# Hippogriff/prifit

Measured on AMD Instinct MI355X. Metric: shapes/sec (fwd+bwd) B=24x2048 pts, PointNet++-MSG+ellipsoid fit, higher is better.
Workload: dtype f32; 1 GPU; configs[2]: PointNet++-MSG + mean-shift(10 it, <=25 clusters) + ellipsoid fit + convex loss, B=24x2048 per GPU, fwd+bwd+Adam; global_batch=24, points=2048, parallelism=dp1, cloud=blobs, embedding=clustered, backbone_grad_param=sa1.conv_blocks.0.0.weight, launch=eager

## Files before the change

include/prifit_hip.h:

```cpp
#ifndef PRIFIT_HIP_H
#define PRIFIT_HIP_H

#include <stdint.h>

#ifdef __cplusplus
extern "C" {
#endif

#define PRIFIT_OK 0
#define PRIFIT_EINVAL (-1)
#define PRIFIT_ELAUNCH (-2)

#define PRIFIT_ABI_VERSION 802
int prifit_version(const char **arch);


int prifit_fps(const float *xyz, int B, int N, int npoint, const int64_t *start_idx,
               int64_t *out_idx, float *new_xyz, void *stream);

int prifit_ball_query(const float *xyz, const float *new_xyz, int B, int N, int S, int R,
                      const float *radius2, const int *nsample, void *const *out, int idx64,
                      void *stream);

int prifit_three_nn(const float *xyz1, const float *xyz2, int B, int N, int S, int32_t *idx,
                    float *dist, float *weight, void *stream);

int prifit_square_distance(const float *src, const float *dst, int B, int S, int N, float *out,
                           void *stream);


int prifit_group_gather(const float *feat, const float *xyz, const float *new_xyz,
                        const int32_t *idx, int B, int N, int S, int K, int C, int order,
                        int ld_out, float *out, void *stream);

int prifit_group_scatter_add(const float *gout, int ld_gout, int col0, const int32_t *idx, int B,
                             int N, int S, int K, int C, float *dfeat, void *stream);

int prifit_pack_cols(const float *w, int rows, int src_cols, const int32_t *map, int dst_cols, float *out, void *stream);
int prifit_unpack_cols(const float *g, int rows, int dst_cols, const int32_t *inv_off, const int32_t *inv_idx, int src_cols,
                       float *gw, void *stream);
int prifit_pack_cols_max_jobs(void);
int prifit_pack_cols_multi(int njobs, const float *const *w, const int32_t *rows, const int32_t *src_cols, const int32_t *const *map,
                           const int32_t *dst_cols, float *const *out, void *stream);
int prifit_unpack_cols_multi(int njobs, const float *const *g, const int32_t *rows, const int32_t *dst_cols, const int32_t *const *inv_off,
                             const int32_t *const *inv_idx, const int32_t *src_cols, float *const *gw, void *stream);

int prifit_three_interpolate(const float *points2, const int32_t *idx, const float *weight, int B,
                             int N, int S, int C, int ld_out, int col0, float *out, void *stream);

int prifit_three_interpolate_bwd(const float *gout, int ld_gout, int col0, const int32_t *idx,
                                 const float *weight, int B, int N, int S, int C, float *dpoints2,
                                 void *stream);
int prifit_fp_rows(const float *points2, const int32_t *idx, const float *weight, const float *points1, int B, int N, int S, int D2,
                   int D1, int kp, float *out, void *stream);


#define PRIFIT_GEMM_NT 0
#define PRIFIT_GEMM_NN 1
#define PRIFIT_GEMM_TN 2
#define PRIFIT_EPI_NONE 0
#define PRIFIT_EPI_CHORD 1
#define PRIFIT_EPI_MSKERNEL 2
#define PRIFIT_EPI_MSBWD 3

int prifit_gemm_f32(int layout, int M, int N, int K, const float *A, long long lda, long long strideA,
                    const float *B, long long ldb, long long strideB, float *C, long long ldc,
                    long long strideC, int batch, int splitk, const float *a_scale,
                    const float *a_shift, const float *b_scale, const float *b_shift,
                    const float *bias, long long bias_batch_stride, float *col_stats, int epilogue,
                    const float *epi_batch_scalar, const float *epi_aux, long long ld_aux,
                    long long stride_aux, const float *epi_row_add, float *a_rowsum, int accumulate, void *stream);

int prifit_chord_sym_f32(const float *A, long long lda, long long strideA, float *C, long long ldc, long long strideC,
                         int n, int K, int batch, unsigned long long *owner_key, void *stream);
int prifit_chord_sym_mask(const float *A, long long lda, long long strideA, const float *thr, uint32_t *mask, int n, int K, int batch,
                          unsigned long long *owner_key, void *stream);
int prifit_gram_sym_f32(const float *A, long long lda, long long strideA, float *C, long long ldc, long long strideC, int n, int K,
                        int batch, void *stream);

int prifit_gemm_pool_f32(int M, int N, int K, const float *A, long long lda, const float *W, long long ldb, float *Y,
                         long long ldc, const float *a_scale, const float *a_shift, const float *bias, float *col_stats,
                         float *cand, void *stream);
int prifit_gemm_pool_supported(int M, int N, int K);

int prifit_gemm_stream_f32(int layout, int M, int N, int K, const float *A, long long lda, const float *B,
                           long long ldb, float *C, long long ldc, const float *a_scale, const float *a_shift,
                           const float *bias, float *col_stats, void *stream);
int prifit_gemm_stream_supported(int layout, int M, int N, int K);
int prifit_gemm_stream_slabs(int M, int K);

int prifit_gemm_dual_nn_f32(int M, int N, int K1, int K2, const float *A1, const float *A2, long long lda,
                            long long strideA, const float *B1, const float *B2, long long ldb, long long strideB,
                            float *C, long long ldc, long long strideC, int batch, int splitk, int accumulate,
                            void *stream);

int prifit_gemm_dgrad_bnred_f32(int M, int N, int K, const float *dY, long long lda, const float *W, long long ldb,
// ... 334 lines not shown
long long prifit_chamfer_nn_workspace_floats(int B, int NA, int NB);
int prifit_chamfer_nn_fwd(const float *a, const float *b, const int32_t *na, const int32_t *nb, int B, int NA, int NB,
                          float *d2, int32_t *idx, float *workspace, void *stream);
int prifit_chamfer_nn_bwd(const float *a, const float *b, const int32_t *na, const int32_t *nb, int B, int NA, int NB,
                          const int32_t *idx, const float *g, float *ga, float *gb, int accumulate_b, void *stream);

long long prifit_atlas_workspace_floats(int num_charts, int B, int P, int backward);
int prifit_atlas_fwd(const void *const *params, const float *z, const float *grid, int num_charts, int B, int P, int training,
                     float eps, float momentum, float *out, float *workspace, void *stream);
int prifit_atlas_bwd(const void *const *params, const float *z, const float *grid, int num_charts, int B, int P, int training,
                     const float *gout, const float *out, const float *fwd_workspace, float *workspace, float *gz,
                     float *gparams, void *stream);


int prifit_knn_topk(const float *G, const float *xx, int B, int N, int k, int32_t *idx, void *stream);
int prifit_knn3_supported(int N, int k);
int prifit_knn3_topk(const float *x, int B, int N, int k, int32_t *idx, void *stream);

int prifit_edge_gather(const float *x, const int32_t *idx, int B, int N, int C, int k, int ld_out,
                       float *out, void *stream);
int prifit_edge_scatter(const float *gout, int ld_gout, const int32_t *idx, int B, int N, int C, int k,
                        float *dx, void *stream);

int prifit_comm_unique_id_bytes(void);
int prifit_comm_in_process(void);
int prifit_comm_unique_id(void *out);
int prifit_comm_init(void **comm, int nranks, int rank, const void *unique_id);
int prifit_allreduce_flat(float *buf, long long count, void *comm, void *stream);
int prifit_comm_destroy(void *comm);

int prifit_adam_flat_alignment(void);
int prifit_adam_flat(float *params, float *exp_avg, float *exp_avg_sq, const float *const *grads, const int32_t *offsets,
                     const int32_t *lengths, int nparams, long long total, const int32_t *step_in, int32_t *step_out, float lr,
                     float beta1, float beta2, float eps, float weight_decay, const int32_t *skip, void *stream);
int prifit_sgd_flat(float *params, float *momentum_buf, const float *const *grads, const int32_t *offsets, const int32_t *lengths,
                    int nparams, long long total, const int32_t *step_in, int32_t *step_out, float lr, float momentum,
                    float dampening, float weight_decay, int nesterov, const int32_t *skip, void *stream);

int prifit_affine_points(const float *src, int B, int M, int C, const float *affine, const int32_t *subset, int n_subset,
                         float *dst_cl, float *dst_cf, float *dst_sub, void *stream);

int prifit_seg_metrics(const float *scores, long long ld, const long long *target, int B, int N, int P,
                       const int32_t *cat_of_label, int restricted, long long *pred, int32_t *shape_cat, int32_t *inter,
                       int32_t *uni, long long *totals, void *stream);


int prifit_fold_bn_max_jobs(void);
int prifit_fold_bn(int njobs, const float *const *W, const int32_t *cout, const int32_t *kin, const float *const *bias,
                   const float *const *gamma, const float *const *beta, const float *const *mean, const float *const *var,
                   const float *eps, const long long *w_off, const int32_t *ldw, const long long *b_off, float *flat,
                   long long flat_len, void *stream);

int prifit_mlp_chain_pool_supported(int C0, int C1, int C2, int pool_K);
long long prifit_mlp_chain_pool_workspace(int G, int pool_K, int C0, int C1, int C2);
int prifit_mlp_chain_pool_f32(const float *X, long long ldx, int G, int pool_K, int C0, int C1, int C2, const float *W1,
                              long long ldw1, const float *b1, const float *W2, long long ldw2, const float *b2, float *out,
                              long long ldo, float *workspace, void *stream);

int prifit_mlp_chain_rows_supported(int K0, int L, const int32_t *widths);
long long prifit_mlp_chain_rows_workspace(long long P, int K0, int L, const int32_t *widths);
int prifit_mlp_chain_rows_f32(const float *X, long long ldx, long long P, int K0, int L, const int32_t *widths,
                              const float *const *W, const long long *ldw, const float *const *b, float *scores, long long lds,
                              int32_t *labels, const int32_t *cat_of_label, const int32_t *shape_cat, int rows_per_shape,
                              float *workspace, void *stream);


int prifit_pack_bf16_max_jobs(void);
int prifit_pack_bf16_multi(int njobs, const float *const *w, const int32_t *rows, const int32_t *cols, const int32_t *ldw,
                           const int32_t *order, uint16_t *const *out, void *stream);

int prifit_mlp_chain_pool_bf16_supported(int C0, int C1, int C2, int pool_K);
long long prifit_mlp_chain_pool_bf16_workspace(int G, int pool_K, int C0, int C1, int C2);
int prifit_mlp_chain_pool_bf16(const float *X, long long ldx, int G, int pool_K, int C0, int C1, int C2, const uint16_t *W1,
                               long long ldw1, const float *b1, const uint16_t *W2, long long ldw2, const float *b2, float *out,
                               long long ldo, float *workspace, void *stream);

int prifit_mlp_chain_rows_bf16_supported(int K0, int L, const int32_t *widths);
long long prifit_mlp_chain_rows_bf16_workspace(long long P, int K0, int L, const int32_t *widths);
int prifit_mlp_chain_rows_bf16(const float *X, long long ldx, long long P, int K0, int L, const int32_t *widths,
                               const uint16_t *const *W, const long long *ldw, const float *const *b, float *scores, long long lds,
                               int32_t *labels, const int32_t *cat_of_label, const int32_t *shape_cat, int rows_per_shape,
                               float *workspace, void *stream);

#ifdef __cplusplus
}
#endif
#endif
```

prifit_amd/build.py:

```python
import os
import subprocess
import sys
from concurrent.futures import ThreadPoolExecutor

HERE = os.path.dirname(os.path.abspath(__file__))
ROOT = os.path.dirname(HERE)
CSRC = os.path.join(HERE, "csrc")
LIBDIR = os.path.join(HERE, "lib")
LIB = os.path.join(LIBDIR, "libprifit_hip.so")
OBJDIR = os.path.join(HERE, "build")
ARCH = "gfx950"

SOURCES = {
    "pointops.hip": ["-ffp-contract=off"],
    "sa_group.hip": ["-ffp-contract=off"],
    "gemm.hip": [],
    "gemm_stream.hip": [],
    "gemm_stream_bwd.hip": [],
    "pool_alg.hip": [],
    "sa_gather_bwd.hip": [],
    "bn.hip": [],
    "meanshift.hip": [],
    "meanshift_fused.hip": [],
    "meanshift_rows.hip": [],
    "meanshift_split.hip": [],
    "fit.hip": [],
    "fit_glue.hip": [],
    "chamfer.hip": ["-ffp-contract=off"],
    "atlas.hip": [],
    "optim.hip": [],
    "augment.hip": ["-ffp-contract=off"],
    "seg_metrics.hip": [],
    "infer.hip": [],
    "infer_bf16.hip": [],
    "edge_conv.hip": [],
    "dgcnn.hip": ["-ffp-contract=off"],
    "comm.hip": [],
}
COMMON = ["-O3", "-std=c++17", "-fPIC", "--offload-arch=" + ARCH, "-I" + os.path.join(ROOT, "include"),
          "-I" + CSRC, "-Wall", "-Wno-unused-function"] + os.environ.get("PRIFIT_BUILD_DEFS", "").split()


def _hipcc():
    for c in (os.environ.get("HIPCC"), "/opt/rocm/bin/hipcc", "hipcc"):
        if c and (os.path.isabs(c) and os.path.exists(c) or not os.path.isabs(c)):
            return c
    raise RuntimeError("hipcc not found")


def _stale(target, deps):
    if not os.path.exists(target):
        return True
    t = os.path.getmtime(target)
    return any(os.path.getmtime(d) > t for d in deps)


def build_library(force=False, verbose=False):
    import fcntl
    os.makedirs(LIBDIR, exist_ok=True)
    os.makedirs(OBJDIR, exist_ok=True)
    with open(os.path.join(LIBDIR, ".build.lock"), "w") as lock:
        fcntl.flock(lock, fcntl.LOCK_EX)
        try:
            return _build_locked(force, verbose)
        finally:
            fcntl.flock(lock, fcntl.LOCK_UN)


def _build_locked(force, verbose):
    headers = [os.path.join(CSRC, f) for f in os.listdir(CSRC) if f.endswith(".h")]
    headers.append(os.path.join(ROOT, "include", "prifit_hip.h"))
    hipcc = _hipcc()
    jobs = []
    objs = []
    for src, extra in SOURCES.items():
        s = os.path.join(CSRC, src)
        o = os.path.join(OBJDIR, src.replace(".hip", ".o"))
        objs.append(o)
        if force or _stale(o, [s] + headers):
            jobs.append([hipcc] + COMMON + extra + ["-c", s, "-o", o])

    def run(cmd):
        if verbose:
            print(" ".join(cmd), flush=True)
        r = subprocess.run(cmd, capture_output=True, text=True)
        if r.returncode != 0:
            raise RuntimeError("hipcc failed:\n%s\n%s" % (" ".join(cmd), r.stderr))
        if verbose and r.stderr.strip():
            print(r.stderr)

    if jobs:
        with ThreadPoolExecutor(max_workers=min(4, len(jobs))) as ex:
            list(ex.map(run, jobs))
    if jobs or force or _stale(LIB, objs):
        tmp = LIB + ".tmp.%d" % os.getpid()
        run([hipcc, "-shared", "-fPIC", "--offload-arch=" + ARCH, "-o", tmp] + objs + ["-ldl"])
        os.replace(tmp, LIB)
    return LIB


if __name__ == "__main__":
    print(build_library(force="--force" in sys.argv, verbose=True))
```

prifit_amd/nn_ops.py:

```python
import collections
import ctypes
import os
import types

import torch

from . import profiler
from . import arena as zero_pool
from ._lib import call, cur_stream, dll, ptr, query

NT, NN, TN = 0, 1, 2
EPI_NONE, EPI_CHORD, EPI_MSKERNEL, EPI_MSBWD = 0, 1, 2, 3
_LL = ctypes.c_longlong
_F = ctypes.c_float
_D = ctypes.c_double


def _rows_per_slab():
    return query("prifit_reduce_rows_per_slab")


_STREAM = os.environ.get("PRIFIT_GEMM_STREAM", "1") != "0"
_FUSE_RED = os.environ.get("PRIFIT_FUSE_BN_REDUCE", "1") != "0"
_FUSE_POOL_FWD = os.environ.get("PRIFIT_FUSE_POOL_FWD", "1") != "0"
# ... 200 lines not shown
             ptr(sc1), ptr(sh1), ptr(mu1), ptr(is1), ptr(rslab), cur_stream())
    return G_prev, ly.dW, rslab, None


def _route_direct0(ly, route):
    if not ly.need_dW:
        return None, None, None, None
    P, Cout, G, fe, dev = ly.P, ly.Cout, ly.G, ly.front, ly.dev
    nblk = int(max(1, min(1024, (P + 1023) // 1024)))
    part = torch.empty(nblk, Cout, fe.D + 3, dtype=torch.float32, device=dev)
    if route.kernel == "gather":
        with profiler.span("sa_first_layer_dw", 4.0 * P * (Cout + 1)):
            call("prifit_sa_first_layer_dw_bn_gather", ptr(G), ptr(fe.U), ptr(fe.Vc), ptr(ly.scale), ptr(ly.shift),
                 ptr(ly.ca), ptr(ly.cb), ptr(ly.cd), ptr(fe.idx), ptr(fe.xyz), ptr(fe.new_xyz),
                 ptr(fe.feat), fe.B, fe.N, fe.S, fe.K, Cout, fe.D, int(fe.feat_first), nblk, ptr(part), cur_stream())
    else:
        with profiler.span("sa_first_layer_dw", 4.0 * P * (2 * Cout + 1)):
            call("prifit_sa_first_layer_dw_bn", ptr(G), ptr(ly.Y), ptr(ly.scale), ptr(ly.shift), ptr(ly.ca), ptr(ly.cb), ptr(ly.cd),
                 ptr(fe.idx), ptr(fe.xyz), ptr(fe.new_xyz), ptr(fe.feat), fe.B, fe.N, fe.S, fe.K, Cout,
                 fe.D, int(fe.feat_first), nblk, ptr(part), cur_stream())
    return None, slab_sum(part), None, None


def _route_gather0(ly, route):
    P, Cout, G, fe, dev = ly.P, ly.Cout, ly.G, ly.front, ly.dev
    Bq, Nq, Sq, Kq = fe.B, fe.N, fe.S, fe.K
    if route.kernel == "csr":
        Uq, Vq = fe.U.detach().contiguous(), fe.Vc.detach().contiguous()
        E = Sq * Kq
        offs = torch.empty(Bq, Nq + 1, dtype=torch.int32, device=dev)
        lst, pos, own = (torch.empty(Bq, E, dtype=torch.int32, device=dev) for _ in range(3))
        wsd = torch.empty(query("prifit_gather_linear_bwd_csr_workspace", Bq, Sq, Kq, Cout), dtype=torch.float64, device=dev)
        dU = torch.empty(Bq, Nq, Cout, dtype=torch.float32, device=dev)
        dVc = torch.empty(Bq, Sq, Cout, dtype=torch.float32, device=dev)
        with profiler.span("gather_linear_bwd", 4.0 * (2.0 * P * Cout + 4.0 * P + 2.0 * (Bq * Nq + Bq * Sq) * Cout)):
            call("prifit_list_csr", ptr(fe.idx), Bq, Nq, E, ptr(offs), ptr(lst), ptr(pos), ptr(own), cur_stream())
            call("prifit_gather_linear_bwd_csr", ptr(G), ptr(Uq), ptr(Vq), ptr(ly.bias0), ptr(ly.scale), ptr(ly.shift),
                 ptr(ly.ca), ptr(ly.cb), ptr(ly.cd), ptr(fe.idx), ptr(offs), ptr(lst), ptr(own), Bq, Nq, Sq, Kq, Cout, ptr(dU),
                 ptr(dVc), ptr(wsd), cur_stream())
    else:
        dU = zero_pool.zeros(Bq, Nq, Cout, device=dev)
        dVc = zero_pool.zeros(Bq, Sq, Cout, device=dev)
        with profiler.span("gather_linear_bwd", 4.0 * (2.0 * P * Cout + P + (Bq * Nq + Bq * Sq) * Cout)):
            call("prifit_gather_linear_bwd_bn", ptr(G), ptr(ly.Y), ptr(ly.scale), ptr(ly.shift), ptr(ly.ca), ptr(ly.cb), ptr(ly.cd),
                 ptr(fe.idx), Bq, Nq, Sq, Kq, Cout, ptr(dU), ptr(dVc), cur_stream())
    return None, dU, None, dVc


def _route_plain(ly, route):
    P, Cout, Kin, G, W, Yp, dev = ly.P, ly.Cout, ly.Kin, ly.G, ly.W, ly.Yp, ly.dev
    dY = torch.empty(P, Cout, dtype=torch.float32, device=dev)
    if ly.pooled:
        call("prifit_pool_bwd_apply", ptr(G), _LL(G.stride(0)), ptr(ly.Y), _LL(Cout), ptr(ly.arg), ptr(ly.scale), ptr(ly.shift),
             ptr(ly.ca), ptr(ly.cb), ptr(ly.cd), P // ly.pool_K, ly.pool_K, Cout, 0, _F(0.0), ptr(dY), _LL(Cout), cur_stream())
    else:
        call("prifit_bn_relu_bwd_apply", ptr(G), _LL(G.stride(0)), ptr(ly.Y), _LL(Cout), ptr(ly.scale), ptr(ly.shift),
             ptr(ly.ca), ptr(ly.cb), ptr(ly.cd), P, Cout, 0, _F(0.0), ptr(dY), _LL(Cout), cur_stream())
    if route.name == "preact0":
        return dY, None, None, None
    dW = _weight_grad(dY, P, Cout, Yp, Kin, ly.aff_p, out=ly.dW) if ly.need_dW else None
    db = dY.sum(dim=0) if ly.want_db else None
    G_prev = None if route.kernel is None else torch.empty(P, Kin, dtype=torch.float32, device=dev)
    rslab = None
    if route.red:
        (sc1, sh1), (mu1, is1) = ly.aff_p, ly.stats_p
    if route.kernel == "gemm":
        gemm(NN, P, Kin, Cout, dY, Cout, W, Kin, G_prev, Kin)
    elif route.kernel == "stream":
        rslab = torch.empty(query("prifit_gemm_stream_slabs", P, Cout), 2, Kin, dtype=torch.float32, device=dev)
        with profiler.span(profiler.tag("gemm_stream_nn", P, Kin, Cout, 0), 4.0 * (P * Cout + 2 * P * Kin + Kin * Cout)):
            call("prifit_gemm_stream_dgrad_f32", P, Kin, Cout, ptr(dY), _LL(Cout), ptr(W), _LL(Kin), ptr(G_prev),
                 _LL(Kin), ptr(Yp), _LL(Yp.stride(0)), ptr(sc1), ptr(sh1), ptr(mu1), ptr(is1), ptr(rslab), cur_stream())
    elif route.kernel == "tiled":
        t = query("prifit_gemm_stats_tile_m", P, Kin)
        rslab = torch.empty((P + t - 1) // t, 2, Kin, dtype=torch.float32, device=dev)
        with profiler.span(profiler.tag("gemm_nn_bn%d" % _bn_tile(Kin), P, Kin, Cout, "red"), 2.0 * P * Kin * Cout):
            call("prifit_gemm_dgrad_bnred_f32", P, Kin, Cout, ptr(dY), _LL(Cout), ptr(W), _LL(Kin), ptr(G_prev),
                 _LL(Kin), ptr(Yp), _LL(Yp.stride(0)), ptr(sc1), ptr(sh1), ptr(mu1), ptr(is1), ptr(rslab), cur_stream())
    return G_prev, dW, rslab, db


_ROUTES = {"pool": _route_pool, "bn": _route_bn, "norows": _fused_bwd, "direct0": _route_direct0,
           "gather0": _route_gather0, "preact0": _route_plain, "plain": _route_plain}


def _eval_coeffs(gamma, beta, rmean, rvar, eps):
    invstd = torch.rsqrt(rvar + eps)
    mean = rmean.clone()
    scale = gamma * invstd
    return scale, beta - mean * scale, mean, invstd


FrontEnd = collections.namedtuple("FrontEnd", "mode slab idx B N S K D xyz new_xyz feat feat_first U Vc",
                                  defaults=(None,) * 12)


def _mlp_tensors(convs, bns, first_weight):
    ts = []
    for i, (conv, bn) in enumerate(zip(convs, bns)):
        w = first_weight if i == 0 else conv.weight.reshape(conv.weight.shape[0], -1)
        ts += [w, conv.bias, bn.weight, bn.bias, bn.running_mean, bn.running_var]
    return ts


def front_end_args(cfg, convs, bns, front):
    cfg["front"] = front
    if front.mode == "gather":
        return cfg, _mlp_tensors(convs, bns, front.U) + [front.Vc]
    if front.mode in ("direct", "norows"):
        return cfg, _mlp_tensors(convs, bns, convs[0].weight.reshape(convs[0].weight.shape[0], -1))
    ts = _mlp_tensors(convs, bns, None)
    ts[1] = None
    return cfg, ts


class SharedMLPFn(torch.autograd.Function):

    @staticmethod
    def forward(ctx, x, cfg, *tensors):
        L = len(tensors) // 6
        front = cfg.get("front")
        mode = "plain" if front is None else front.mode
        nr = front if mode == "norows" else None
        if nr is not None:
            P, dev = nr.B * nr.S * nr.K, nr.U.device
        else:
            P, K0 = x.shape
            dev = x.device
        training = cfg["training"]
        Ys, affines, stats_saved, Ws = [], [], [], []
        prev, prev_aff = x, None
        cand = None
        for l in range(L):
            W, b, gamma, beta, rmean, rvar = tensors[6 * l:6 * l + 6]
            preact = l == 0 and front is not None
            if preact:
                W, Cout, Kin, Y = None, (nr.U.shape[-1] if nr is not None else x.shape[1]), 0, x
            else:
                W = W.contiguous()
                Cout, Kin = W.shape
                assert Kin == (nr.U.shape[-1] if (l == 1 and nr is not None) else prev.shape[1]), (Kin, l)
                Y = torch.empty(P, Cout, dtype=torch.float32, device=dev)
            if preact:
                slab = front.slab
            elif not training:
                gemm(NT, P, Cout, Kin, prev, prev.stride(0), W, Kin, Y, Cout, a_affine=prev_aff, bias=b)
            elif l == 1 and nr is not None:
                slab = torch.empty(query("prifit_gemm_stream_slabs", P, Kin), 2, Cout, dtype=torch.float32, device=dev)
                with profiler.span(profiler.tag("gemm_stream_nt", P, Cout, Kin, "gather"), 4.0 * (P * Cout + P + Cout * Kin)):
                    call("prifit_gemm_stream_gather_f32", P, Cout, ptr(nr.idx), ptr(nr.U), ptr(nr.Vc), nr.N, nr.S,
                         nr.K, ptr(W), _LL(Kin), ptr(Y), _LL(Cout), ptr(prev_aff[0]), ptr(prev_aff[1]), ptr(b), ptr(slab),
                         cur_stream())
            else:
                aligned = prev.stride(0) % 4 == 0 and prev.data_ptr() % 16 == 0 and W.data_ptr() % 16 == 0
                tile_m = query("prifit_gemm_stats_tile_m", P, Cout)
                nslab = gemm_stats_slabs(P, Cout, Kin) if aligned else (P + tile_m - 1) // tile_m
                slab = torch.empty(nslab, 2, Cout, dtype=torch.float32, device=dev)
                kernel = _forward_kernel(l == L - 1, cfg["pool_K"], aligned, prev_aff is not None, P, Cout, Kin)
                if kernel == "gemm":
                    gemm(NT, P, Cout, Kin, prev, prev.stride(0), W, Kin, Y, Cout, a_affine=prev_aff, bias=b, stats=slab)
                else:
                    cand = torch.empty(P // 32, 4, Cout, dtype=torch.float32, device=dev)
                    if kernel == "stream_pool":
                        with profiler.span(profiler.tag("gemm_stream_nt", P, Cout, Kin, 1), 4.0 * (P * Kin + P * Cout + Cout * Kin)):
                            call("prifit_gemm_stream_pool_f32", P, Cout, Kin, ptr(prev), _LL(prev.stride(0)), ptr(W), _LL(Kin),
                                 ptr(Y), _LL(Cout), ptr(prev_aff[0]), ptr(prev_aff[1]), ptr(b), ptr(slab), ptr(cand), cur_stream())
                    else:
                        with profiler.span(profiler.tag("gemm_nt_bn128", P, Cout, Kin, "pool"), 2.0 * P * Cout * Kin):
                            call("prifit_gemm_pool_f32", P, Cout, Kin, ptr(prev), _LL(prev.stride(0)), ptr(W), _LL(Kin), ptr(Y),
                                 _LL(Cout), ptr(prev_aff[0]), ptr(prev_aff[1]), ptr(b), ptr(slab), ptr(cand), cur_stream())
            if training:
                scale, shift, mean, invstd = torch.empty(4, Cout, dtype=torch.float32, device=dev).unbind(0)
                call("prifit_bn_finalize", ptr(slab), slab.shape[0], Cout, _D(float(P)), ptr(gamma), ptr(beta),
                     _F(cfg["eps"]), _F(cfg["momentum"][l]), ptr(rmean), ptr(rvar), ptr(scale), ptr(shift),
                     ptr(mean), ptr(invstd), cur_stream())
            else:
                scale, shift, mean, invstd = _eval_coeffs(gamma, beta, rmean, rvar, cfg["eps"])
            Ys.append(Y)
            Ws.append(W)
            affines.append((scale, shift))
            stats_saved.append((mean, invstd))
            prev, prev_aff = Y, (scale, shift)
        CL = Ys[-1].shape[1]
        pool_K = cfg["pool_K"]
        arg = None
        if pool_K:
            G = P // pool_K
            out = cfg.get("pool_out")
            if out is None:
                out = torch.empty(G, CL, dtype=torch.float32, device=dev)
            elif tuple(out.shape) != (G, CL) or out.stride(1) != 1 or out.dtype != torch.float32 or out.device != dev:
                raise ValueError("pool_out must be a [G, C] fp32 column window on the input's device")
            arg = torch.empty(G, CL, dtype=torch.int32, device=dev)
            if cand is not None:
                call("prifit_pool_from_candidates", ptr(cand), ptr(prev_aff[0]), ptr(prev_aff[1]), G, pool_K, CL, 0, _F(0.0),
                     ptr(out), _LL(out.stride(0)), ptr(arg), None, cur_stream())
            else:
                call("prifit_pool_fwd", ptr(Ys[-1]), _LL(CL), ptr(prev_aff[0]), ptr(prev_aff[1]), G, pool_K, CL, 0, _F(0.0),
                     ptr(out), _LL(out.stride(0)), ptr(arg), cur_stream())
        else:
            out = torch.empty(P, CL, dtype=torch.float32, device=dev)
            call("prifit_affine_relu", ptr(Ys[-1]), _LL(CL), ptr(prev_aff[0]), ptr(prev_aff[1]), P, CL, 0, _F(0.0),
                 ptr(out), _LL(CL), cur_stream())
        ctx.cfg = {k: v for k, v in cfg.items() if k not in ("front", "pool_out")}
        ctx.mode, ctx.front = mode, front
        ctx.L = L
        ctx.P, ctx.dev = P, dev
        assert nr is None or (training and L >= 3 and Ys[0] is None)
        ctx.saved = (x, Ys, Ws, affines, stats_saved, arg)
        ctx.bias0 = tensors[1]
        return out

    @staticmethod
    def backward(ctx, gout):
        cfg, L, needs = ctx.cfg, ctx.L, ctx.needs_input_grad
        x, Ys, Ws, affines, stats_saved, arg = ctx.saved
        training, pool_K = cfg["training"], cfg["pool_K"]
        P, dev, front, mode = ctx.P, ctx.dev, ctx.front, ctx.mode
        if not (pool_K and L > 1 and gout.dim() == 2 and gout.stride(1) == 1 and gout.stride(0) % 4 == 0 and
                gout.data_ptr() % 16 == 0):
            gout = gout.contiguous()
        rps = _rows_per_slab()
        grads = [None] * (6 * L)
        wslots, total = {}, 0
        for l in range(L):
            if Ws[l] is None:
                continue
            n = Ws[l].numel() if needs[2 + 6 * l] else 0
            nb = Ws[l].shape[0] if (training and needs[2 + 6 * l + 1]) else 0
            wslots[l] = (total, n, total + n, nb)
            total += n + nb
        arena = zero_pool.zeros(total, device=dev) if total else None
        G_in = gout
        fused_red = None
        for l in range(L - 1, -1, -1):
            Y, W = Ys[l], Ws[l]
            Cout, Kin = W.shape if W is not None else ((front.U.shape[-1] if Y is None else Y.shape[1]), 0)
            scale, shift = affines[l]
            mean, invstd = stats_saved[l]
            pooled = l == L - 1 and bool(pool_K)
            dgamma, dbeta, ca, cb, cd = torch.empty(5, Cout, dtype=torch.float32, device=dev).unbind(0)
            if pooled:
                prs = query("prifit_pool_reduce_groups_per_slab")
                slab = torch.empty((P // pool_K + prs - 1) // prs, 2, Cout, dtype=torch.float32, device=dev)
                call("prifit_pool_bwd_reduce", ptr(G_in), _LL(G_in.stride(0)), ptr(Y), _LL(Cout), ptr(arg), ptr(scale),
                     ptr(shift), ptr(mean), ptr(invstd), P // pool_K, pool_K, Cout, 0, _F(0.0), ptr(slab), cur_stream())
            elif fused_red is not None:
                slab = fused_red
            else:
                slab = torch.empty((P + rps - 1) // rps, 2, Cout, dtype=torch.float32, device=dev)
                call("prifit_bn_relu_bwd_reduce", ptr(G_in), _LL(G_in.stride(0)), ptr(Y), _LL(Cout), ptr(scale),
                     ptr(shift), ptr(mean), ptr(invstd), P, Cout, 0, _F(0.0), ptr(slab), cur_stream())
            call("prifit_bn_bwd_finalize", ptr(slab), slab.shape[0], Cout, _D(float(P)), int(training), ptr(scale),
                 ptr(mean), ptr(invstd), ptr(dgamma), ptr(dbeta), ptr(ca), ptr(cb), ptr(cd), cur_stream())
            route = _backward_route(
                l, L, P, Cout, Kin, pool_K, training, mode, needs[2 + 6 * l], needs[0],
                g_dense=G_in.stride(0) == Cout and G_in.data_ptr() % 16 == 0, g_contig=G_in.is_contiguous(),
                below_ld4=l > 0 and Ys[l - 1] is not None and Ys[l - 1].stride(0) % 4 == 0,
                N0=front.N if mode == "gather" else 0)
            wo, wn, bo, nb = wslots.get(l, (0, 0, 0, 0))
            Yp, aff_p, stats_p = (Ys[l - 1], affines[l - 1], stats_saved[l - 1]) if l > 0 else (x, None, None)
            ly = types.SimpleNamespace(
                P=P, Cout=Cout, Kin=Kin, dev=dev, pooled=pooled, pool_K=pool_K, arg=arg, G=G_in, Y=Y, W=W, scale=scale, shift=shift,
                ca=ca, cb=cb, cd=cd, Yp=Yp, aff_p=aff_p, stats_p=stats_p, front=front, bias0=ctx.bias0,
                dW=arena[wo:wo + wn].view(Cout, Kin) if wn else None, need_dW=needs[2 + 6 * l],
                want_db=needs[3 + 6 * l] and not training)
            G_in, grads[6 * l], fused_red, extra = _ROUTES[route.name](ly, route)
            if needs[3 + 6 * l]:
                grads[6 * l + 1] = (arena[bo:bo + nb] if training else extra) if l in wslots else zero_pool.zeros(Cout, device=dev)
            grads[6 * l + 2] = dgamma
            grads[6 * l + 3] = dbeta
        return (G_in, None) + tuple(grads) + ((extra,) if mode == "gather" else ())


class GatherLinearFn(torch.autograd.Function):

    @staticmethod
    def forward(ctx, U, Vc, bias, idx, training):
        U, Vc, idx = U.contiguous(), Vc.contiguous(), idx.contiguous()
        B, N, C = U.shape
        _, S, K = idx.shape
        assert Vc.shape == (B, S, C) and idx.dtype == torch.int32, (Vc.shape, idx.dtype)
        P = B * S * K
        Y = torch.empty(P, C, dtype=torch.float32, device=U.device)
        rps = _rows_per_slab()
        slab = torch.empty((P + rps - 1) // rps, 2, C, dtype=torch.float32, device=U.device)
        with profiler.span("gather_linear", 4.0 * B * (N * C + S * C + S * K + S * K * C)):
            call("prifit_gather_linear_fwd", ptr(U), ptr(Vc), ptr(bias), ptr(idx), B, N, S, K, C, ptr(Y), ptr(slab),
                 cur_stream())
        ctx.save_for_backward(idx)
        ctx.meta = (B, N, S, K, C, training)
        ctx.mark_non_differentiable(slab)
        return Y, slab

    @staticmethod
    def backward(ctx, gY, _gslab):
        (idx,) = ctx.saved_tensors
        B, N, S, K, C, training = ctx.meta
        gY = gY.contiguous()
        dU = zero_pool.zeros(B, N, C, device=gY.device)
        dVc = torch.empty(B, S, C, dtype=torch.float32, device=gY.device)
        call("prifit_gather_linear_bwd", ptr(gY), ptr(idx), B, N, S, K, C, ptr(dU), ptr(dVc), cur_stream())
        db = None
        if ctx.needs_input_grad[2]:
            db = zero_pool.zeros(C, device=gY.device) if training else gY.sum(dim=0)
        return dU, dVc, db, None, None


def _ptr_array(tensors):
    return (ctypes.c_void_p * len(tensors))(*[None if t is None else t.data_ptr() for t in tensors])


def sa_group_supported(N, nsamples, widths):
    return (N <= 2048 and 1 <= len(nsamples) <= 4 and sum(nsamples) <= 320 and
            all(16 <= c <= 128 and (c & (c - 1)) == 0 for c in widths))


def _sa_group_launch(mode, xyz, new_xyz, feat, feat_first, radii, nsamples, widths, Ws, Us, Vcs, biases,
                     feat_xyz=False, rows=None):
    import numpy as np

    B, N, _ = xyz.shape
    S = new_xyz.shape[1]
    R = len(radii)
    dev = xyz.device
    q = query("prifit_sa_group_queries_per_slab", B, S)
    nslab = B * ((S + q - 1) // q)
    rows = [True] * R if rows is None else list(rows)
    assert mode == 1 or all(rows)
    Ys = [torch.empty(B * S * k, c, dtype=torch.float32, device=dev) if keep else None
          for k, c, keep in zip(nsamples, widths, rows)]
    slabs = [torch.empty(nslab, 2, c, dtype=torch.float32, device=dev) for c in widths]
    idxs = [torch.empty(B, S, k, dtype=torch.int32, device=dev) for k in nsamples]
    r2 = (ctypes.c_float * R)(*[float(np.float32(r ** 2)) for r in radii])
    ns = (ctypes.c_int * R)(*[int(k) for k in nsamples])
    wd = (ctypes.c_int * R)(*[int(c) for c in widths])
    D = 0 if feat is None else feat.shape[-1]
    work = B * (12.0 * (N + S) + sum(4.0 * S * k * (1 + (c if keep else 0)) for k, c, keep in zip(nsamples, widths, rows)) +
                (sum(4.0 * (N + S) * c for c in widths) if mode == 1 else 4.0 * N * D))
    with profiler.span("sa_group_linear", work):
        call("prifit_sa_group_linear_fwd", ptr(xyz), ptr(new_xyz), B, N, S, R, r2, ns, wd, mode, ptr(feat), D,
             int(feat_first), int(feat_xyz), _ptr_array(Ws) if Ws else None, _ptr_array(Us) if Us else None,
             _ptr_array(Vcs) if Vcs else None, _ptr_array(biases), _ptr_array(Ys), _ptr_array(slabs), _ptr_array(idxs),
             cur_stream())
    return Ys, slabs, idxs


def sa_point_tables(first_convs, feats, xyz, new_xyz, feat_first):
    B, N, _ = xyz.shape
    S = new_xyz.shape[1]
    D = 0 if feats is None else feats.shape[-1]
    R = len(first_convs)
    Ws = [c.weight.detach().reshape(c.weight.shape[0], -1).contiguous() for c in first_convs]
    bs = [None if c.bias is None else c.bias.detach().contiguous() for c in first_convs]
# ... 40 lines not shown
                gY = gY.contiguous()
                P = B * S * K
                nblk = int(max(1, min(1024, (P + 1023) // 1024)))
                part = torch.empty(nblk, C, D + 3, dtype=torch.float32, device=gY.device)
                with profiler.span("sa_first_layer_dw", 4.0 * P * (C + 1)):
                    call("prifit_sa_first_layer_dw", ptr(gY), ptr(idxs[r]), ptr(xyz), ptr(new_xyz), ptr(feat), B, N, S,
                         K, C, D, int(feat_first), nblk, ptr(part), cur_stream())
                dW = slab_sum(part)
                if has_bias[r]:
                    db = zero_pool.zeros(C, device=gY.device) if training else gY.sum(dim=0)
            grads += [dW, db]
        return (None, None, None, None) + tuple(grads)


class SAGroupGatherFn(torch.autograd.Function):

    @staticmethod
    def forward(ctx, xyz, new_xyz, meta, *tensors):
        radii, nsamples, training = meta
        Us = [u.contiguous() for u in tensors[0::3]]
        Vcs = [v.contiguous() for v in tensors[1::3]]
        bs = [None if b is None else b.contiguous() for b in tensors[2::3]]
        widths = [u.shape[-1] for u in Us]
        Ys, slabs, idxs = _sa_group_launch(1, xyz, new_xyz, None, True, radii, nsamples, widths, None, Us, Vcs, bs)
        ctx.save_for_backward(*idxs)
        ctx.meta = (xyz.shape[0], xyz.shape[1], new_xyz.shape[1], nsamples, widths, training, [b is not None for b in bs])
        out = []
        for y, sl in zip(Ys, slabs):
            out += [y, sl]
        ctx.mark_non_differentiable(*slabs)
        return tuple(out)

    @staticmethod
    def backward(ctx, *gouts):
        idxs = ctx.saved_tensors
        B, N, S, nsamples, widths, training, has_bias = ctx.meta
        grads = []
        for r, (K, C) in enumerate(zip(nsamples, widths)):
            gY = gouts[2 * r]
            dU = dVc = db = None
            if gY is not None:
                gY = gY.contiguous()
                dU = zero_pool.zeros(B, N, C, device=gY.device)
                dVc = torch.empty(B, S, C, dtype=torch.float32, device=gY.device)
                call("prifit_gather_linear_bwd", ptr(gY), ptr(idxs[r]), B, N, S, K, C, ptr(dU), ptr(dVc), cur_stream())
                if has_bias[r]:
                    db = zero_pool.zeros(C, device=gY.device) if training else gY.sum(dim=0)
            grads += [dU, dVc, db]
        return (None, None, None) + tuple(grads)


def _few_rows_splitk(M, N, K):
    if M > 128 or K < 256:
        return 1
    tiles = max(1, (N + 127) // 128)
    return int(max(1, min(256 // tiles, K // 64)))


class LinearFn(torch.autograd.Function):

    @staticmethod
    def forward(ctx, x, W, b):
        x = x.contiguous()
        W = W.contiguous()
        P, Kin = x.shape
        Cout = W.shape[0]
        sk = _few_rows_splitk(P, Cout, Kin)
        if sk > 1:
            Y = zero_pool.zeros(P, Cout, device=x.device)
            gemm(NT, P, Cout, Kin, x, Kin, W, Kin, Y, Cout, bias=b, splitk=sk)
        else:
            Y = torch.empty(P, Cout, dtype=torch.float32, device=x.device)
            gemm(NT, P, Cout, Kin, x, Kin, W, Kin, Y, Cout, bias=b)
        ctx.save_for_backward(x, W)
        return Y

    @staticmethod
    def backward(ctx, gy):
        x, W = ctx.saved_tensors
        gy = gy.contiguous()
        P, Kin = x.shape
        Cout = W.shape[0]
        dx = dW = db = None
        if ctx.needs_input_grad[0]:
            sk = _few_rows_splitk(P, Kin, Cout)
            if sk > 1:
                dx = zero_pool.zeros(P, Kin, device=x.device)
                gemm(NN, P, Kin, Cout, gy, Cout, W, Kin, dx, Kin, splitk=sk)
            else:
                dx = torch.empty(P, Kin, dtype=torch.float32, device=x.device)
                gemm(NN, P, Kin, Cout, gy, Cout, W, Kin, dx, Kin)
        if ctx.needs_input_grad[1]:
            dW = _weight_grad(gy, P, Cout, x, Kin, None)
        if ctx.needs_input_grad[2]:
            if Cout % 4 == 0 and gy.data_ptr() % 16 == 0:
                db = torch.empty(Cout, dtype=torch.float32, device=x.device)
                ws = torch.empty(query("prifit_col_sum_workspace", P, Cout), dtype=torch.float32, device=x.device)
                call("prifit_col_sum", ptr(gy), _LL(Cout), P, Cout, ptr(db), ptr(ws), cur_stream())
            else:
                db = gy.sum(dim=0)
        return dx, dW, db


class CrossEntropyFn(torch.autograd.Function):

    @staticmethod
    def forward(ctx, x, target):
        if x.stride(1) != 1:
            x = x.contiguous()
        target = target.contiguous()
        P, C = x.shape
        lse = torch.empty(P, dtype=torch.float32, device=x.device)
        ws = torch.empty(query("prifit_cross_entropy_workspace"), dtype=torch.float32, device=x.device)
        loss = torch.empty(2, dtype=torch.float32, device=x.device)
        call("prifit_cross_entropy_fwd", ptr(x), _LL(x.stride(0)), ptr(target), _LL(P), C, ptr(lse), ptr(ws), ptr(loss), cur_stream())
        ctx.save_for_backward(x, target, lse, loss)
        return loss[0]

    @staticmethod
    def backward(ctx, g):
        x, target, lse, loss = ctx.saved_tensors
        P, C = x.shape
        dx = torch.empty(P, C, dtype=torch.float32, device=x.device)
        g = g.reshape(1).to(torch.float32).contiguous()
        call("prifit_cross_entropy_bwd", ptr(x), _LL(x.stride(0)), ptr(target), ptr(lse), ptr(g), ptr(loss[1:]), _LL(P), C, ptr(dx),
             _LL(C), cur_stream())
        return dx, None


_GATHER_BWD_CSR = os.environ.get("PRIFIT_GATHER_BWD_CSR", "1") != "0"
_CE_KERNEL = os.environ.get("PRIFIT_CE_KERNEL", "1") != "0"


def cross_entropy(x, target):
    if _CE_KERNEL and x.is_cuda and x.dim() == 2 and x.dtype == torch.float32 and x.shape[1] <= 64 and target.dim() == 1 and target.dtype == torch.int64:
        return CrossEntropyFn.apply(x, target)
    return torch.nn.functional.cross_entropy(x, target)


class GroupGatherFn(torch.autograd.Function):

    @staticmethod
    def forward(ctx, feat, xyz, new_xyz, idx, order, ld_out):
        from . import ops

        out = ops.group_gather(feat, xyz, new_xyz, idx, order=order, ld_out=ld_out)
        ctx.save_for_backward(idx)
        ctx.meta = (feat.shape, order) if feat is not None else None
        return out

    @staticmethod
    def backward(ctx, gout):
        from . import ops

        if ctx.meta is None or not ctx.needs_input_grad[0]:
            return (None,) * 6
        (idx,) = ctx.saved_tensors
        (B, N, C), order = ctx.meta
        gout = gout.contiguous()
        dfeat = ops.group_scatter_add(gout, 0 if order == 0 else 3, idx, B, N, C)
        return dfeat, None, None, None, None, None


class ConcatWindowsFn(torch.autograd.Function):

    @staticmethod
    def forward(ctx, wide, *windows):
        ctx.widths = [w.shape[1] for w in windows]
        return wide.view_as(wide)

    @staticmethod
    def backward(ctx, g):
        outs, c0 = [], 0
        for wd in ctx.widths:
            outs.append(g[:, c0:c0 + wd])
# ... 53 lines not shown
```

Before: 1649 shapes/s.

## Batch small-MLP backward layers into one native call with optional side-stream dW

```diff
diff --git a/include/prifit_hip.h b/include/prifit_hip.h
--- a/include/prifit_hip.h
+++ b/include/prifit_hip.h
@@ -11,7 +11,7 @@
 #define PRIFIT_EINVAL (-1)
 #define PRIFIT_ELAUNCH (-2)
 
-#define PRIFIT_ABI_VERSION 802
+#define PRIFIT_ABI_VERSION 803
 int prifit_version(const char **arch);
 
 
@@ -512,6 +512,27 @@
                                int32_t *labels, const int32_t *cat_of_label, const int32_t *shape_cat, int rows_per_shape,
                                float *workspace, void *stream);
 
+
+int prifit_fork(void *main_stream);
+int prifit_join(void *main_stream);
+long long prifit_side_stream(void *main_stream);
+
+typedef struct PrifitMlpBwdLayer {
+    long long P, Cout, Kin;
+    long long reduce, finalize, apply, nslab, training;
+    long long dw_splitk, fork, dA, da_splitk;
+    const float *G;
+    long long ldg;
+    const float *Y, *scale, *shift, *mean, *invstd;
+    float *slab, *coef, *dY;
+    const float *Yp;
+    long long ldyp;
+    const float *scale_p, *shift_p, *mean_p, *invstd_p, *W;
+    float *dW, *Gp, *rslab;
+} PrifitMlpBwdLayer;
+int prifit_mlp_bwd_layer_bytes(void);
+int prifit_mlp_bwd_small(const PrifitMlpBwdLayer *layers, int n, int fork, int join, int *forked, void *stream);
+
 #ifdef __cplusplus
 }
 #endif
diff --git a/prifit_amd/build.py b/prifit_amd/build.py
--- a/prifit_amd/build.py
+++ b/prifit_amd/build.py
@@ -36,6 +36,7 @@
     "edge_conv.hip": [],
     "dgcnn.hip": ["-ffp-contract=off"],
     "comm.hip": [],
+    "fork.hip": [],
 }
 COMMON = ["-O3", "-std=c++17", "-fPIC", "--offload-arch=" + ARCH, "-I" + os.path.join(ROOT, "include"),
           "-I" + CSRC, "-Wall", "-Wno-unused-function"] + os.environ.get("PRIFIT_BUILD_DEFS", "").split()
diff --git a/prifit_amd/csrc/fork.hip b/prifit_amd/csrc/fork.hip
--- /dev/null
+++ b/prifit_amd/csrc/fork.hip
@@ -0,0 +1,141 @@
+#include <mutex>
+
+#include "common.h"
+
+namespace {
+
+constexpr int kMaxDevices = 64;
+constexpr int kRing = 16;
+
+struct Side {
+    hipStream_t stream = nullptr;
+    hipEvent_t ev[kRing] = {};
+    int next = 0;
+    bool ok = false;
+};
+
+std::mutex g_mu;
+Side g_side[kMaxDevices];
+
+Side *side_of_current_device()
+{
+    int dev = -1;
+    if (hipGetDevice(&dev) != hipSuccess || dev < 0 || dev >= kMaxDevices) return nullptr;
+    Side &s = g_side[dev];
+    if (!s.ok) {
+        if (hipStreamCreateWithFlags(&s.stream, hipStreamNonBlocking) != hipSuccess) return nullptr;
+        for (int i = 0; i < kRing; ++i)
+            if (hipEventCreateWithFlags(&s.ev[i], hipEventDisableTiming | hipEventDisableSystemFence) != hipSuccess) return nullptr;
+        s.ok = true;
+    }
+    return &s;
+}
+
+bool capturing(hipStream_t st)
+{
+    hipStreamCaptureStatus status = hipStreamCaptureStatusNone;
+    if (hipStreamIsCapturing(st, &status) != hipSuccess) {
+        (void)hipGetLastError();
+        return true;
+    }
+    return status != hipStreamCaptureStatusNone;
+}
+
+int order_behind(Side &s, hipStream_t from, hipStream_t to)
+{
+    hipEvent_t e = s.ev[s.next];
+    s.next = (s.next + 1) % kRing;
+    if (hipEventRecord(e, from) != hipSuccess) return PRIFIT_ELAUNCH;
+    if (hipStreamWaitEvent(to, e, 0) != hipSuccess) return PRIFIT_ELAUNCH;
+    return PRIFIT_OK;
+}
+
+}
+
+extern "C" {
+
+int prifit_fork(void *main_stream)
+{
+    hipStream_t st = as_stream(main_stream);
+    if (capturing(st)) return PRIFIT_OK;
+    std::lock_guard<std::mutex> lock(g_mu);
+    Side *s = side_of_current_device();
+    if (!s) return PRIFIT_ELAUNCH;
+    return order_behind(*s, st, s->stream);
+}
+
+int prifit_join(void *main_stream)
+{
+    hipStream_t st = as_stream(main_stream);
+    if (capturing(st)) return PRIFIT_OK;
+    std::lock_guard<std::mutex> lock(g_mu);
+    Side *s = side_of_current_device();
+    if (!s) return PRIFIT_ELAUNCH;
+    return order_behind(*s, s->stream, st);
+}
+
+long long prifit_side_stream(void *main_stream)
+{
+    if (capturing(as_stream(main_stream))) return (long long)(intptr_t)main_stream;
+    std::lock_guard<std::mutex> lock(g_mu);
+    Side *s = side_of_current_device();
+    return (long long)(intptr_t)(s ? (void *)s->stream : main_stream);
+}
+
+int prifit_mlp_bwd_layer_bytes(void) { return (int)sizeof(PrifitMlpBwdLayer); }
+
+int prifit_mlp_bwd_small(const PrifitMlpBwdLayer *layers, int n, int fork, int join, int *forked, void *stream)
+{
+    if (forked) *forked = 0;
+    if (!layers || n < 0) return PRIFIT_EINVAL;
+    const bool may_fork = fork && !capturing(as_stream(stream));
+    void *side = may_fork ? (void *)(intptr_t)prifit_side_stream(stream) : stream;
+    int nforked = 0, rc = PRIFIT_OK;
+    for (int i = 0; i < n && rc == PRIFIT_OK; ++i) {
+        const PrifitMlpBwdLayer &L = layers[i];
+        const int P = (int)L.P, Cout = (int)L.Cout, Kin = (int)L.Kin;
+        if (L.P <= 0 || L.P > 0x7fffffffLL || Cout <= 0 || Kin < 0 || !L.dY) {
+            rc = PRIFIT_EINVAL;
+            break;
+        }
+        float *coef = L.coef;
+        if (L.reduce)
+            rc = prifit_bn_relu_bwd_reduce(L.G, L.ldg, L.Y, Cout, L.scale, L.shift, L.mean, L.invstd, P, Cout, 0, 0.0f, L.slab,
+                                           stream);
+        if (rc == PRIFIT_OK && L.finalize)
+            rc = prifit_bn_bwd_finalize(L.slab, (int)L.nslab, Cout, (double)L.P, (int)L.training, L.scale, L.mean, L.invstd, coef,
+                                        coef + Cout, coef + 2 * Cout, coef + 3 * Cout, coef + 4 * Cout, stream);
+        if (rc == PRIFIT_OK && L.apply)
+            rc = prifit_bn_relu_bwd_apply(L.G, L.ldg, L.Y, Cout, L.scale, L.shift, coef + 2 * Cout, coef + 3 * Cout,
+                                          coef + 4 * Cout, P, Cout, 0, 0.0f, L.dY, Cout, stream);
+        if (rc == PRIFIT_OK && L.dw_splitk >= 1) {
+            void *st = stream;
+            if (may_fork && L.fork && side != stream) {
+                rc = prifit_fork(stream);
+                if (rc == PRIFIT_OK) {
+                    st = side;
+                    ++nforked;
+                }
+            }
+            if (rc == PRIFIT_OK)
+                rc = prifit_gemm_f32(PRIFIT_GEMM_TN, Cout, Kin, P, L.dY, Cout, 0, L.Yp, L.ldyp, 0, L.dW, Kin, 0, 1, (int)L.dw_splitk,
+                                     nullptr, nullptr, L.scale_p, L.shift_p, nullptr, 0, nullptr, 0 , nullptr,
+                                     nullptr, 0, 0, nullptr, nullptr, L.dw_splitk > 1 ? 1 : 0, st);
+        }
+        if (rc == PRIFIT_OK && L.dA == 1)
+            rc = prifit_gemm_f32(PRIFIT_GEMM_NN, P, Kin, Cout, L.dY, Cout, 0, L.W, Kin, 0, L.Gp, Kin, 0, 1, (int)L.da_splitk, nullptr,
+                                 nullptr, nullptr, nullptr, nullptr, 0, nullptr, 0 , nullptr, nullptr, 0, 0,
+                                 nullptr, nullptr, L.da_splitk > 1 ? 1 : 0, stream);
+        else if (rc == PRIFIT_OK && L.dA == 2)
+            rc = prifit_gemm_dgrad_bnred_f32(P, Kin, Cout, L.dY, Cout, L.W, Kin, L.Gp, Kin, L.Yp, L.ldyp, L.scale_p, L.shift_p,
+                                             L.mean_p, L.invstd_p, L.rslab, stream);
+    }
+    if (nforked && (join || rc != PRIFIT_OK)) {
+        const int jr = prifit_join(stream);
+        if (rc == PRIFIT_OK) rc = jr;
+    }
+    if (forked) *forked = nforked;
+    return rc;
+}
+
+}
diff --git a/prifit_amd/nn_ops.py b/prifit_amd/nn_ops.py
--- a/prifit_amd/nn_ops.py
+++ b/prifit_amd/nn_ops.py
@@ -306,6 +306,50 @@
 
 _ROUTES = {"pool": _route_pool, "bn": _route_bn, "norows": _fused_bwd, "direct0": _route_direct0,
            "gather0": _route_gather0, "preact0": _route_plain, "plain": _route_plain}
+
+
+
+_DW_FORK = os.environ.get("PRIFIT_DW_FORK", "0") != "0"
+
+_FORK_MAX_ROWS = 65536
+
+fork_stats = {"calls": 0, "forked": 0}
+
+
+class _BwdLayer(ctypes.Structure):
+    _fields_ = ([(n, _LL) for n in ("P", "Cout", "Kin", "reduce", "finalize", "apply", "nslab", "training", "dw_splitk", "fork",
+                                    "dA", "da_splitk")] +
+                [("G", ctypes.c_void_p), ("ldg", _LL)] +
+                [(n, ctypes.c_void_p) for n in ("Y", "scale", "shift", "mean", "invstd", "slab", "coef", "dY", "Yp")] +
+                [("ldyp", _LL)] +
+                [(n, ctypes.c_void_p) for n in ("scale_p", "shift_p", "mean_p", "invstd_p", "W", "dW", "Gp", "rslab")])
+
+
+def _dw_splitk(P, Cout, Kin):
+    return _splitk_for(P, ((Cout + 127) // 128) * ((Kin + 127) // 128))
+
+
+def _small_products(P, Cout, Kin, need_dW, dA):
+    if P > _FORK_MAX_ROWS or profiler._enabled:
+        return False
+    if need_dW and _STREAM and query("prifit_gemm_stream_tn_supported", Cout, Kin, P):
+        return False
+    return not (dA == "gemm" and _stream_ok(NN, P, Kin, Cout))
+
+
+def _run_small_bwd(layers, join):
+    if ctypes.sizeof(_BwdLayer) != query("prifit_mlp_bwd_layer_bytes"):
+        raise RuntimeError("PrifitMlpBwdLayer: the binding's layout differs from the library's")
+    arr = (_BwdLayer * len(layers))()
+    for d, f in zip(arr, layers):
+        for k, v in f.items():
+            setattr(d, k, v.data_ptr() if isinstance(v, torch.Tensor) else v)
+    forked = ctypes.c_int(0)
+    call("prifit_mlp_bwd_small", ctypes.addressof(arr), len(layers), int(_DW_FORK), int(join), ctypes.addressof(forked),
+         cur_stream())
+    fork_stats["calls"] += 1
+    fork_stats["forked"] += forked.value
+    return forked.value
 
 
 def _eval_coeffs(gamma, beta, rmean, rvar, eps):
@@ -457,12 +501,47 @@
         arena = zero_pool.zeros(total, device=dev) if total else None
         G_in = gout
         fused_red = None
+        pending, keep, unjoined = [], [], 0
         for l in range(L - 1, -1, -1):
             Y, W = Ys[l], Ws[l]
             Cout, Kin = W.shape if W is not None else ((front.U.shape[-1] if Y is None else Y.shape[1]), 0)
             scale, shift = affines[l]
             mean, invstd = stats_saved[l]
             pooled = l == L - 1 and bool(pool_K)
+            route = _backward_route(
+                l, L, P, Cout, Kin, pool_K, training, mode, needs[2 + 6 * l], needs[0],
+                g_dense=G_in.stride(0) == Cout and G_in.data_ptr() % 16 == 0, g_contig=G_in.is_contiguous(),
+                below_ld4=l > 0 and Ys[l - 1] is not None and Ys[l - 1].stride(0) % 4 == 0,
+                N0=front.N if mode == "gather" else 0)
+            wo, wn, bo, nb = wslots.get(l, (0, 0, 0, 0))
+            Yp, aff_p, stats_p = (Ys[l - 1], affines[l - 1], stats_saved[l - 1]) if l > 0 else (x, None, None)
+            if (route.name == "plain" and route.kernel != "stream" and not pool_K and not (needs[3 + 6 * l] and not training) and
+                    _small_products(P, Cout, Kin, needs[2 + 6 * l], route.kernel)):
+                coef = torch.empty(5, Cout, dtype=torch.float32, device=dev)
+                slab = fused_red if fused_red is not None else torch.empty((P + rps - 1) // rps, 2, Cout, dtype=torch.float32, device=dev)
+                dY = torch.empty(P, Cout, dtype=torch.float32, device=dev)
+                dW = arena[wo:wo + wn].view(Cout, Kin) if wn else None
+                Gp = None if route.kernel is None else torch.empty(P, Kin, dtype=torch.float32, device=dev)
+                rslab = None
+                if route.kernel == "tiled":
+                    t = query("prifit_gemm_stats_tile_m", P, Kin)
+                    rslab = torch.empty((P + t - 1) // t, 2, Kin, dtype=torch.float32, device=dev)
+                (sc1, sh1), (mu1, is1) = (aff_p, stats_p) if l > 0 else ((None, None), (None, None))
+                pending.append(dict(
+                    P=P, Cout=Cout, Kin=Kin, reduce=int(fused_red is None), finalize=1, apply=1, nslab=slab.shape[0],
+                    training=int(training), dw_splitk=_dw_splitk(P, Cout, Kin) if dW is not None else 0,
+                    fork=int(dW is not None and Gp is not None), dA={None: 0, "gemm": 1, "tiled": 2}[route.kernel], da_splitk=1,
+                    G=G_in, ldg=G_in.stride(0), Y=Y, scale=scale, shift=shift, mean=mean, invstd=invstd, slab=slab, coef=coef, dY=dY,
+                    Yp=Yp, ldyp=Yp.stride(0), scale_p=sc1, shift_p=sh1, mean_p=mu1, invstd_p=is1, W=W, dW=dW, Gp=Gp, rslab=rslab))
+                keep += [G_in, slab, coef, dY, Gp, rslab]
+                G_in, grads[6 * l], fused_red = Gp, dW, rslab
+                if needs[3 + 6 * l]:
+                    grads[6 * l + 1] = arena[bo:bo + nb]
+                grads[6 * l + 2], grads[6 * l + 3] = coef[0], coef[1]
+                continue
+            if pending:
+                unjoined += _run_small_bwd(pending, join=False)
+                pending = []
             dgamma, dbeta, ca, cb, cd = torch.empty(5, Cout, dtype=torch.float32, device=dev).unbind(0)
             if pooled:
                 prs = query("prifit_pool_reduce_groups_per_slab")
@@ -477,13 +556,6 @@
                      ptr(shift), ptr(mean), ptr(invstd), P, Cout, 0, _F(0.0), ptr(slab), cur_stream())
             call("prifit_bn_bwd_finalize", ptr(slab), slab.shape[0], Cout, _D(float(P)), int(training), ptr(scale),
                  ptr(mean), ptr(invstd), ptr(dgamma), ptr(dbeta), ptr(ca), ptr(cb), ptr(cd), cur_stream())
-            route = _backward_route(
-                l, L, P, Cout, Kin, pool_K, training, mode, needs[2 + 6 * l], needs[0],
-                g_dense=G_in.stride(0) == Cout and G_in.data_ptr() % 16 == 0, g_contig=G_in.is_contiguous(),
-                below_ld4=l > 0 and Ys[l - 1] is not None and Ys[l - 1].stride(0) % 4 == 0,
-                N0=front.N if mode == "gather" else 0)
-            wo, wn, bo, nb = wslots.get(l, (0, 0, 0, 0))
-            Yp, aff_p, stats_p = (Ys[l - 1], affines[l - 1], stats_saved[l - 1]) if l > 0 else (x, None, None)
             ly = types.SimpleNamespace(
                 P=P, Cout=Cout, Kin=Kin, dev=dev, pooled=pooled, pool_K=pool_K, arg=arg, G=G_in, Y=Y, W=W, scale=scale, shift=shift,
                 ca=ca, cb=cb, cd=cd, Yp=Yp, aff_p=aff_p, stats_p=stats_p, front=front, bias0=ctx.bias0,
@@ -494,6 +566,11 @@
                 grads[6 * l + 1] = (arena[bo:bo + nb] if training else extra) if l in wslots else zero_pool.zeros(Cout, device=dev)
             grads[6 * l + 2] = dgamma
             grads[6 * l + 3] = dbeta
+        if pending:
+            unjoined += _run_small_bwd(pending, join=False)
+        if unjoined:
+            call("prifit_join", cur_stream())
+        del keep
         return (G_in, None) + tuple(grads) + ((extra,) if mode == "gather" else ())
 
 
@@ -700,7 +777,13 @@
         P, Kin = x.shape
         Cout = W.shape[0]
         dx = dW = db = None
-        if ctx.needs_input_grad[0]:
+        if ctx.needs_input_grad[0] and ctx.needs_input_grad[1] and _small_products(P, Cout, Kin, True, "gemm"):
+            sk, skw = _few_rows_splitk(P, Kin, Cout), _dw_splitk(P, Cout, Kin)
+            dx = (zero_pool.zeros if sk > 1 else torch.empty)(P, Kin, dtype=torch.float32, device=x.device)
+            dW = (zero_pool.zeros if skw > 1 else torch.empty)(Cout, Kin, dtype=torch.float32, device=x.device)
+            _run_small_bwd([dict(P=P, Cout=Cout, Kin=Kin, dw_splitk=skw, fork=1, dA=1, da_splitk=sk, dY=gy, Yp=x, ldyp=Kin, W=W,
+                                 dW=dW, Gp=dx)], join=True)
+        elif ctx.needs_input_grad[0]:
             sk = _few_rows_splitk(P, Kin, Cout)
             if sk > 1:
                 dx = zero_pool.zeros(P, Kin, device=x.device)
@@ -708,7 +791,7 @@
             else:
                 dx = torch.empty(P, Kin, dtype=torch.float32, device=x.device)
                 gemm(NN, P, Kin, Cout, gy, Cout, W, Kin, dx, Kin)
-        if ctx.needs_input_grad[1]:
+        if ctx.needs_input_grad[1] and dW is None:
             dW = _weight_grad(gy, P, Cout, x, Kin, None)
         if ctx.needs_input_grad[2]:
             if Cout % 4 == 0 and gy.data_ptr() % 16 == 0:
```

After: 1644 shapes/s. About the same (-0.3%).
